# ethz-asl/multipoint

Measured on AMD Instinct MI355X. Metric: image-pairs/sec (detect+desc+match) @ 480x640, higher is better.
Workload: dtype f32

## Files before the change

### multipoint_amd/csrc/api.hip

```cpp
#include "host.h"

using namespace mp_host;

namespace {

bool debug_switch(const char* key, int* value = nullptr, int dflt = 1)
{
    const char* e = getenv("MP_DEBUG");
    if (!e) return false;
    const size_t kl = std::strlen(key);
    for (const char* q = e; *q;) {
        while (*q == ',' || *q == ' ') ++q;
        const char* end = q;
        while (*end && *end != ',') ++end;
        if ((size_t)(end - q) >= kl && std::strncmp(q, key, kl) == 0 && (q[kl] == '=' || q + kl == end || q[kl] == ' ')) {
            if (value) *value = q[kl] == '=' ? atoi(q + kl + 1) : dflt;
            return true;
        }
        q = end;
    }
    return false;
}

int kfd_num_xcc(const char* bus_id)
// ... 7 lines not shown
        FILE* f = fopen(path, "r");
        if (!f) { if (node > 8) break; else continue; }
        char key[64]; unsigned long long val = 0, loc = ~0ull, domain = 0, xcc = 0, simd = 0;
        while (fscanf(f, "%63s %llu", key, &val) == 2) {
            if (!strcmp(key, "location_id")) loc = val;
            else if (!strcmp(key, "domain")) domain = val;
            else if (!strcmp(key, "num_xcc")) xcc = val;
            else if (!strcmp(key, "simd_count")) simd = val;
        }
        fclose(f);
        if (simd > 0 && loc == want && domain == dom) return (int)xcc;
    }
    return 0;
}

}

extern "C" {

const char* mp_version(void) { return "multipoint_hip 0.1 (gfx950)"; }

const char* mp_last_error(const mp_handle* h) { return h ? h->err.c_str() : g_create_error.c_str(); }

int mp_device_shape(const mp_handle* h, int* compute_units, int* xcds, int* persistent_workgroups)
{
    if (!h) return MP_EINVAL;
    if (compute_units) *compute_units = h->ncu;
    if (xcds) *xcds = 1 << h->xcd_shift;
    if (persistent_workgroups) *persistent_workgroups = (int)persistent_grid(1ll << 40, h->ncu, h->xcd_shift);
    return MP_OK;
}

int mp_create(mp_handle** out, int device)
{
    mp_handle* h = nullptr;
    if (!out) return fail(h, MP_EINVAL, "mp_create: out is NULL");
    *out = nullptr;
    int ndev = 0;
    MP_HIP(hipGetDeviceCount(&ndev));
    if (device < 0 || device >= ndev)
        return fail(h, MP_EINVAL, "mp_create: device " + std::to_string(device) + " not available (" +
                                      std::to_string(ndev) + " HIP devices visible)");
    MP_HIP(hipSetDevice(device));
    {
        static const char* const legacy[] = {"MP_NO_WINOGRAD", "MP_WINO43", "MP_WINO43_GEN", "MP_NO_FUSE", "MP_NO_FUSE43", "MP_NO_HEAD_FUSE",
            "MP_NO_PLANAR", "MP_PLANAR", "MP_NO_PERSIST", "MP_PERSIST_MIN_ITEMS", "MP_SPLITK_MAX", "MP_F16_NO_RES", "MP_F16_NO_FUSE1",
            "MP_F16_RES_GROUPS", "MP_NCU", "MP_NXCD", "MP_POST_OVERLAP", "MP_NO_VIN", "MP_NO_POOL_FIRST"};
        static bool warned = false;
        for (const char* k : legacy)
            if (!warned && getenv(k)) {
                warned = true;
                fprintf(stderr, "libmultipoint_hip: the environment variable %s is no longer read (nor are the other MP_* kernel switches): "
                                "use MP_DEBUG=key[=value],... -- the keys are listed in csrc/api.hip (debug_switch)\n", k);
            }
    }
    hipDeviceProp_t prop;
    MP_HIP(hipGetDeviceProperties(&prop, device));
    if (std::strncmp(prop.gcnArchName, "gfx950", 6) != 0)
        return fail(h, MP_EINVAL, std::string("mp_create: kernels are built for gfx950 only, device is ") +
                                      prop.gcnArchName);
    int ncu = prop.multiProcessorCount, nxcd = 0;
    {
        char bus[64] = {0};
        if (hipDeviceGetPCIBusId(bus, sizeof bus, device) == hipSuccess) nxcd = kfd_num_xcc(bus);
        if (nxcd <= 0) nxcd = ncu >= 32 ? ncu / 32 : 1;
        int v = 0;
        if (debug_switch("ncu", &v) && v > 0 && v <= ncu) ncu = v;
        if (debug_switch("nxcd", &v) && v > 0) nxcd = v;
    }
    if (ncu < 1 || nxcd < 1 || (nxcd & (nxcd - 1)) != 0 || nxcd > ncu)
        return fail(h, MP_EINVAL, "mp_create: unsupported machine shape: " + std::to_string(ncu) + " compute units in " +
                                      std::to_string(nxcd) + " XCDs (the XCD count must be a power of two <= the CU count)");
    int xcd_shift = 0;
    while ((1 << xcd_shift) < nxcd) ++xcd_shift;
    DebugSwitches d;
    int v = 0;
    d.winograd = !debug_switch("no_winograd");
    if (debug_switch("wino43", &v) && v == 0) d.wino43 = false;
    if (debug_switch("wino43_gen", &v) && v >= 0 && v <= 2) d.wino43_gen = v;
    d.fuse_first = !debug_switch("no_fuse");
    d.fuse43 = !debug_switch("no_fuse43");
    d.head_fuse = !debug_switch("no_head_fuse");
    d.vin = !debug_switch("no_vin");
    d.planar = !debug_switch("no_planar");
    d.xplanar = d.planar && !debug_switch("no_xplanar");
    if (debug_switch("persist_min_items", &v) && v > 0) d.persist = v;
    if (debug_switch("no_persist")) d.persist = 0;
    if (debug_switch("splitk_max", &v) && v >= 1 && v <= 8) d.splitk_max = v;
    d.f16_res = !debug_switch("f16_no_res");
    d.f16_fuse1 = !debug_switch("f16_no_fuse1");
    if (debug_switch("f16_res_groups", &v) && v == 2) d.f16_res_groups = 2;
    mp_handle* hh = new mp_handle(device, ncu, xcd_shift, d);
    if (hipHostMalloc(reinterpret_cast<void**>(&hh->pinned), 4096) != hipSuccess) {
        delete hh;
        return fail(h, MP_ENOMEM, "mp_create: hipHostMalloc failed");
    }
    *out = hh;
    return MP_OK;
}

void mp_destroy(mp_handle* h)
{
    if (!h) return;
    (void)hipSetDevice(h->device);
    int* pinned = h->pinned;
    const std::vector<ProfEntry> events = std::move(h->prof_entries);
    delete h;
    if (pinned) (void)hipHostFree(pinned);
    for (auto& e : events) { (void)hipEventDestroy(e.a); (void)hipEventDestroy(e.b); }
}

int mp_profile_enable(mp_handle* h, int enable)
{
    if (!h) return MP_EINVAL;
    h->prof = enable != 0;
    h->prof_used = 0;
    return MP_OK;
}

int mp_profile_read(mp_handle* h, const char** names, float* ms, double* flop, int capacity, int* n)
{
    if (!h || !n) return MP_EINVAL;
    *n = 0;
    for (size_t i = 0; i < h->prof_used && (int)i < capacity; ++i) {
        ProfEntry& e = h->prof_entries[i];
        MP_HIP(hipEventSynchronize(e.b));
        float t = 0.f;
        MP_HIP(hipEventElapsedTime(&t, e.a, e.b));
        if (names) names[i] = e.name;
        if (ms) ms[i] = t;
        if (flop) flop[i] = e.flop;
        ++*n;
    }
    h->prof_used = 0;
    return MP_OK;
}

}
```

### multipoint_amd/csrc/conv_wino43.hip

```cpp
#include "mp_common.h"
#include "mp_device.h"
#include "mp_tile.h"

#include <algorithm>
#include <type_traits>

MP_TIMING_TABLE(g_timing_q, 256 * 8, mp_debug_read_timing_wino43)
MP_TIMING_HEIGHT(g_timing_q_sel, 480, mp_debug_select_height_wino43)

namespace {

constexpr int NPIX = 18 * 34;
constexpr int UC4 = 4;
constexpr int VB4 = UC4 * 32 * 36;
constexpr int UB4 = UC4 * 64 * 36;
constexpr int NRB = (NPIX + 63) / 64;
constexpr int RB4 = NRB * 64 * 4;
constexpr int SW4 = 8 * 36 * 2;


template <int LEAD = 0>
__device__ __forceinline__ void dma16(const float* sbase, unsigned voff_bytes, unsigned lds_byte)
{
    lds_dma<4, LEAD, 0>(sbase, voff_bytes, lds_byte);
}

template <bool POOL, bool BNF, int TC4, bool F1, bool SPLIT = false, bool VIN = false>
__global__ __launch_bounds__(512, 2) void conv_wino43_kernel(const ConvParams p)
{
    static_assert(!(F1 && SPLIT), "the fused first block is never split");
    static_assert(!(VIN && (F1 || SPLIT)), "pre-transformed input: plain launches only");
    constexpr int TR4 = 32 / TC4;
    constexpr int OY = 4 * TR4, OX = 4 * TC4;
    constexpr int PY = OY + 2, PX = OX + 2;
    static_assert(PY * PX == NPIX, "item shape");
    __shared__ __attribute__((aligned(16))) float Vs[(VIN ? 4 : 2) * VB4];
    __shared__ __attribute__((aligned(16))) float Us[2 * UB4];
    __shared__ __attribute__((aligned(16))) float raw[VIN ? 256 : 3 * RB4 + 256];
    __shared__ __attribute__((aligned(16))) float scr[VIN ? 4 : 8 * SW4];
    __shared__ __attribute__((aligned(16))) float prm[(POOL && !SPLIT ? 6 : 3) * 64];

    const int tid = threadIdx.x;
    const int lane = tid & 63;
    const int wave = __builtin_amdgcn_readfirstlane(tid >> 6);
    const int tb = wave & 1, cb = wave >> 1;
    const int NC = SPLIT ? (p.cin / UC4) >> p.ks_shift : p.cin / UC4;

    const XcdRange xr = xcd_range(p.nitems, p.xcd_shift);
    const int stride = xr.stride, item_end = xr.item_end;
    int item = xr.item;
    if (item >= item_end) return;

    struct Where { int slice, img, y0, x0, tile; const float* in_base; };
    auto decode = [&](int it) __attribute__((always_inline)) -> Where {
        Where w{};
        const int tile = (int)udiv((unsigned)it, p.magic_slices, (unsigned)p.nslices);
        w.slice = it - tile * p.nslices;
        w.tile = tile;
        const int trow = (int)udiv((unsigned)tile, p.magic_tx, (unsigned)p.tiles_x);
        const int tx = tile - trow * p.tiles_x;
        const int bi = (int)udiv((unsigned)trow, p.magic_ty, (unsigned)p.tiles_y);
        const int ty = trow - bi * p.tiles_y;
        w.img = p.img_list ? p.img_list[bi] : bi;
        w.y0 = ty * OY; w.x0 = tx * OX;
        w.in_base = p.in_planar ? p.in + (long long)w.img * (p.cin / 4) * p.H * p.W * 4
                                : p.in + (long long)w.img * p.H * p.W * p.in_cstride + p.in_coff;
        if constexpr (SPLIT)
            w.in_base += (long long)((w.slice & ((1 << p.ks_shift) - 1)) * NC) * (p.in_planar ? (long long)p.H * p.W * 4 : UC4);
        return w;
    };

    const int pix_stride = p.in_planar ? 4 : p.in_cstride;
    const long long unit_stride = p.in_planar ? (long long)p.H * p.W * 4 : UC4;
    const int x_shift = p.in_planar == MP_LAYOUT_XPLANAR ? 2 : 0, x_mask = p.in_planar == MP_LAYOUT_XPLANAR ? 3 : 0;
    const int row_stride = p.W * pix_stride;
    auto pixel_off = [&](int y, int x) __attribute__((always_inline)) -> int {
        return y * row_stride + (x >> x_shift) * pix_stride + (x & x_mask) * p.W;
    };
    unsigned rvoff[2];
    bool roff_rel = false;
    auto raw_offsets = [&](const Where& w) __attribute__((always_inline)) -> const float* {
        const bool interior = (w.y0 >= 1) && (w.y0 + OY < p.H) && (w.x0 >= 1) && (w.x0 + OX < p.W);
        if (interior) {
            if (!roff_rel) {
#pragma unroll
                for (int j = 0; j < 2; ++j) {
                    const int f = (wave + 8 * j) * 64 + lane;
                    const int py = f / PX, px = f - py * PX;
                    rvoff[j] = (f < NPIX) ? (unsigned)pixel_off(py, px + x_mask) * 4u : 0u;
                }
                roff_rel = true;
            }
            return w.in_base + pixel_off(w.y0 - 1, w.x0 - 1 - x_mask);
        }
        roff_rel = false;
#pragma unroll
        for (int j = 0; j < 2; ++j) {
            const int f = (wave + 8 * j) * 64 + lane;
            const int py = f / PX, px = f - py * PX;
            unsigned off = 0;
            if (f < NPIX) {
                const int gy = reflect_clamp(w.y0 + py - 1, p.H), gx = reflect_clamp(w.x0 + px - 1, p.W);
                off = (unsigned)pixel_off(gy, gx) * 4u;
            }
            rvoff[j] = off;
        }
        return w.in_base;
    };
    const unsigned raw_lds = lds_addr(raw), us_lds = lds_addr(Us);
    const unsigned raw_m0 = raw_lds + (unsigned)wave * 1024u;
    const unsigned raw_dummy = raw_lds + 3u * RB4 * 4u;
    auto raw_dma = [&](const float* src, unsigned boff_bytes, int j) __attribute__((always_inline)) {
        const unsigned dst = j == 0 ? raw_m0 + boff_bytes : (wave + 8 < NRB ? raw_m0 + 8192u + boff_bytes : raw_dummy);
        dma16(src, rvoff[j], dst);
    };
    int u_first, u_cnt;
    if constexpr (F1) {
        constexpr int cnt_[8] = {3, 3, 6, 6, 4, 4, 5, 5}, first_[8] = {0, 3, 14, 20, 6, 10, 26, 31};
        u_cnt = 3; u_first = 0;
#pragma unroll
        for (int w = 0; w < 8; ++w) { u_cnt = wave == w ? cnt_[w] : u_cnt; u_first = wave == w ? first_[w] : u_first; }
    } else {
        u_cnt = wave < 4 ? 5 : 4; u_first = wave < 4 ? 5 * wave : 20 + 4 * (wave - 4);
    }
    auto u_dma_site = [&](const float* ub, int buf, int site) __attribute__((always_inline)) {
        if constexpr (VIN) {
#pragma unroll
            for (int i = 3 * site; i < (site ? 5 : 3); ++i) {
                int b = wave + 8 * i;
                b = b < 36 ? b : 35;
                dma16(ub + b * 256, (unsigned)lane * 16u, us_lds + (unsigned)(buf * UB4 + b * 256) * 4u);
            }
            return;
        }
#pragma unroll
        for (int k = 3 * site; k < 3 * site + 3; ++k)
            if (k < u_cnt) {
                const int b = u_first + k;
                dma16<1>(ub + b * 256, (unsigned)lane * 16u, us_lds + (unsigned)(buf * UB4 + b * 256) * 4u);
            }
    };
// ... 315 lines not shown
                    acc[s] = __builtin_amdgcn_mfma_f32_16x16x4f32(af[g % 3][e], bf[g % 3][e], FIRST ? zero4 : acc[s], 0, 0, 0);
                    __builtin_amdgcn_sched_barrier(0);
                    if constexpr (!VIN) { if (e != 2) tf_at(g, e, vb); }
                    if constexpr (F1) prod_at(g, e, vb);
                    if (e == 0) {
                        af[(g + 2) % 3] = *reinterpret_cast<const f32x4*>(g + 2 < 9 ? &ur[4 * (g + 2)] : &urn[4 * (g - 7)]);
                        bf[(g + 2) % 3] = *reinterpret_cast<const f32x4*>(g + 2 < 9 ? &vr[4 * (g + 2)] : &vrn[4 * (g - 7)]);
                    } else if (e == 1) {
                        if (g == 7) u_dma_site(un2, vb, 0);
                        else if (g == 8) u_dma_site(un2, vb, 1);
                        else if (g == 0) { if constexpr (VIN) v_dma(vcur, (vs + 3) & 3, 0); else if constexpr (!F1) raw_dma(rsrc, rd_byte, 0); }
                        else if (g == 1) { if constexpr (VIN) v_dma(vcur, (vs + 3) & 3, 1); else if constexpr (!F1) raw_dma(rsrc, rd_byte, 1); }
                        else if (g == 2) { if constexpr (VIN) v_dma(vcur, (vs + 3) & 3, 2); }
                    } else if (e == 2) {
                        if constexpr (!VIN) tf_at(g, 2, vb);
                    } else {
                        if (g == 6) {
#ifdef MP_TIMING
                            t_b0 = __builtin_amdgcn_s_memtime();
#endif
                            if constexpr (F1) asm volatile("s_waitcnt vmcnt(0) lgkmcnt(0)" ::: "memory");
                            else if constexpr (VIN) asm volatile("s_waitcnt vmcnt(3) lgkmcnt(0)" ::: "memory");
                            else asm volatile("s_waitcnt vmcnt(2) lgkmcnt(0)" ::: "memory");
#ifdef MP_TIMING
                            t_b1 = __builtin_amdgcn_s_memtime();
#endif
                            __syncthreads();
#ifdef MP_TIMING
                            tsum[4] += __builtin_amdgcn_s_memtime() - t_b1;
#endif
                        }
                    }
                    __builtin_amdgcn_sched_barrier(0);
                }
            }
            MP_CLOCK(t_u1);
            MP_CLOCK_ADD(0, t_u0, t_u1);
            MP_CLOCK_ADD(1, t_b0, t_b1);
        };
        auto unit = [&](const int c, auto first_tag, auto vb_tag, auto vs_tag) __attribute__((always_inline)) {
            unit_body(c, first_tag, vb_tag, vs_tag);
            if constexpr (VIN) {
                v_advance();
            } else if constexpr (F1) {
                prod_advance();
            } else {
                ld_advance();
                const unsigned ro = 3u * RB4 * 4u - rd_byte - rt_byte;
                rd_byte = rt_byte; rt_byte = ro;
            }
        };
        using VB0 = std::integral_constant<int, 0>;
        using VB1 = std::integral_constant<int, 1>;
        using VS2 = std::integral_constant<int, 2>;
        using VS3 = std::integral_constant<int, 3>;
        if constexpr (VIN) {
            unit(0, std::true_type{}, VB0{}, VB0{});
            for (int c = 1; c + 3 < NC; c += 4) {
                unit(c, std::false_type{}, VB1{}, VB1{});
                unit(c + 1, std::false_type{}, VB0{}, VS2{});
                unit(c + 2, std::false_type{}, VB1{}, VS3{});
                unit(c + 3, std::false_type{}, VB0{}, VB0{});
            }
            unit(NC - 3, std::false_type{}, VB1{}, VB1{});
            unit(NC - 2, std::false_type{}, VB0{}, VS2{});
            unit(NC - 1, std::false_type{}, VB1{}, VS3{});
        } else {
        unit(0, std::true_type{}, VB0{}, VB0{});
        for (int c = 1; c + 1 < NC; c += 2) {
            unit(c, std::false_type{}, VB1{}, VB1{});
            unit(c + 1, std::false_type{}, VB0{}, VB0{});
        }
        unit(NC - 1, std::false_type{}, VB1{}, VB1{});
        }

        MP_CLOCK(t_e0);
        MP_CLOCK_ADD(3, t_item, t_e0);
        if constexpr (F1) { if (item_next + stride < item_end) patch_dma(decode(item_next + stride), cur_par); }
        const int tl = tb * 16 + (lane & 15);
        const int cl = cb * 16 + 4 * (lane >> 4);
        const f32x4 b4 = *reinterpret_cast<const f32x4*>(&prm[cl]);
        const f32x4 s4 = *reinterpret_cast<const f32x4*>(&prm[64 + cl]);
        const f32x4 t4 = *reinterpret_cast<const f32x4*>(&prm[128 + cl]);
        const int oy = cur.y0 + 4 * (tl / TC4), ox = cur.x0 + 4 * (tl % TC4);
        const int ch0 = (SPLIT ? cur.slice >> p.ks_shift : cur.slice) * 64 + cl;
        const int cs = p.out_cstride;
        constexpr int NO = POOL ? 2 : 4;
        f32x2 keep[NO][NO];
        if constexpr (SPLIT) {
            unsigned long long* const part = reinterpret_cast<unsigned long long*>(p.split_scratch) + (long long)item * (2 * 16 * 512) + tid;
#pragma unroll
            for (int h = 0; h < 2; ++h) {
                f32x2 tcol[4][6];
#pragma unroll
                for (int j = 0; j < 6; ++j) {
                    f32x2 m[6], y[4];
#pragma unroll
                    for (int i = 0; i < 6; ++i) m[i] = f32x2{acc[6 * i + j][2 * h], acc[6 * i + j][2 * h + 1]};
                    at6s(m, y);
#pragma unroll
                    for (int a = 0; a < 4; ++a) tcol[a][j] = y[a];
                }
#pragma unroll
                for (int a = 0; a < 4; ++a) {
                    f32x2 y[4];
                    at6s(tcol[a], y);
#pragma unroll
                    for (int b = 0; b < 4; ++b)
                        part[(h * 16 + a * 4 + b) * 512] = __builtin_bit_cast(unsigned long long, y[b]);
                }
            }
        }
        if constexpr (!SPLIT) {
#pragma unroll
        for (int h = 0; h < 2; ++h) {
            f32x2 tcol[4][6];
            if constexpr (!SPLIT) {
#pragma unroll
            for (int j = 0; j < 6; ++j) {
                f32x2 m[6], y[4];
#pragma unroll
                for (int i = 0; i < 6; ++i) m[i] = f32x2{acc[6 * i + j][2 * h], acc[6 * i + j][2 * h + 1]};
                at6s(m, y);
#pragma unroll
                for (int a = 0; a < 4; ++a) tcol[a][j] = y[a];
            }
            }
            const f32x2 bb = {b4[2 * h], b4[2 * h + 1]}, ss = {s4[2 * h], s4[2 * h + 1]}, tt = {t4[2 * h], t4[2 * h + 1]};
            f32x2 res[NO][NO];
            if constexpr (POOL) {
                const f32x4 g4 = *reinterpret_cast<const f32x4*>(&prm[192 + cl]);
                const f32x4 lo4 = *reinterpret_cast<const f32x4*>(&prm[256 + cl]), hi4 = *reinterpret_cast<const f32x4*>(&prm[320 + cl]);
                const f32x2 gg = {g4[2 * h], g4[2 * h + 1]};
                const f32x2 gb = bb * gg;
                constexpr float A1 = (float)MP_W43_A, A2 = A1 * A1, A3 = A2 * A1, A4 = A2 * A2;
                const f32x2 gk[5] = {gg, gg * f32x2{A1, A1}, gg * f32x2{A2, A2}, gg * f32x2{A3, A3}, gg * f32x2{A4, A4}};
                f32x2 xv[4][4];
#pragma unroll
                for (int a = 0; a < 4; ++a) {
                    f32x2 y[4];
                    at6s(tcol[a], y);
#pragma unroll
                    for (int b = 0; b < 4; ++b) {
                        const int e = (a == 1 ? 1 : a == 2 ? 2 : 0) + (b == 1 ? 1 : b == 2 ? 2 : 0);
                        xv[a][b] = __builtin_elementwise_fma(y[b], gk[e], gb);
                    }
                }
#pragma unroll
                for (int a = 0; a < NO; ++a)
#pragma unroll
                    for (int b = 0; b < NO; ++b) {
                        f32x2 m;
#pragma unroll
                        for (int r = 0; r < 2; ++r)
                            m[r] = fmaxf(fmaxf(xv[2 * a][2 * b][r], xv[2 * a][2 * b + 1][r]), fmaxf(xv[2 * a + 1][2 * b][r], xv[2 * a + 1][2 * b + 1][r]));
                        if (BNF) {
                            m = __builtin_elementwise_fma(m, ss, tt);
                            m = f32x2{relu_bits(m[0]), relu_bits(m[1])};
                        } else {
#pragma unroll
                            for (int r = 0; r < 2; ++r)
                                asm("v_med3_i32 %0, %1, %2, %3" : "=v"(m[r]) : "v"(m[r]), "v"(lo4[2 * h + r]), "v"(hi4[2 * h + r]));
                            m = __builtin_elementwise_fma(m, ss, tt);
                        }
                        res[a][b] = m;
                    }
            } else {
            f32x2 yv[4][4];
#pragma unroll
            for (int a = 0; a < 4; ++a) {
                f32x2 y[4];
                at6s(tcol[a], y);
#pragma unroll
                for (int b = 0; b < 4; ++b) {
                    f32x2 v = w43_add_bias(y[b], a, b, bb);
                    if (BNF) { v = v * ss + tt; v = f32x2{relu_bits(v[0]), relu_bits(v[1])}; }
                    else { v = f32x2{relu_bits(v[0]), relu_bits(v[1])}; v = v * ss + tt; }
                    yv[a][b] = v;
                }
            }
#pragma unroll
            for (int a = 0; a < NO; ++a)
#pragma unroll
                for (int b = 0; b < NO; ++b) res[a][b] = yv[a][b];
            }
            if (h == 0) {
#pragma unroll
                for (int a = 0; a < NO; ++a)
#pragma unroll
                    for (int b = 0; b < NO; ++b) keep[a][b] = res[a][b];
            } else {
                const int Ho = POOL ? p.H >> 1 : p.H, Wo = POOL ? p.W >> 1 : p.W;
                const int py0 = POOL ? oy >> 1 : oy, px0 = POOL ? ox >> 1 : ox;
                const bool xpl = !POOL && p.out_planar == MP_LAYOUT_XPLANAR;
                char* const img_base = reinterpret_cast<char*>(
                    p.out_planar ? p.out + (long long)cur.img * (p.cout / 4) * Ho * Wo * 4
                                 : p.out + (long long)cur.img * Ho * Wo * cs + p.out_coff);
                const unsigned ps = xpl ? (unsigned)Wo * 4u : p.out_planar ? 16u : (unsigned)cs * 4u;
                const unsigned rs = p.out_planar ? (unsigned)Wo * 16u : (unsigned)Wo * ps;
                const unsigned o0 = xpl ? (unsigned)(((ch0 >> 2) * Ho + py0) * Wo * 4 + px0) * 4u
                                  : p.out_planar ? (unsigned)(((ch0 >> 2) * Ho + py0) * Wo + px0) * 16u
                                                 : (unsigned)((py0 * Wo + px0) * cs + ch0) * 4u;
                if (oy < p.H && ox < p.W && ch0 < p.cout) {
#pragma unroll
                    for (int a = 0; a < NO; ++a)
#pragma unroll
                        for (int b = 0; b < NO; ++b) {
                            const f32x4 v = {keep[a][b][0], keep[a][b][1], res[a][b][0], res[a][b][1]};
                            *reinterpret_cast<f32x4*>(img_base + (o0 + (unsigned)a * rs + (unsigned)b * ps)) = v;
                        }
                }
            }
        }
        }
        MP_CLOCK(t_e1);
        MP_CLOCK_ADD(2, t_e0, t_e1);
#ifdef MP_TIMING
        tsum[7] += 1;
        if (!has_next && tid == 0 && t_on)
            for (int i = 0; i < 8; ++i) g_timing_q[blockIdx.x * 8 + i] = tsum[i];
#endif
        if (!has_next) { dma_wait(); return; }
        if (next_slice != cur.slice) {
            __syncthreads();
            load_prm(next_slice);
        }
        item = item_next;
        cur = decode(item);
        cur_par ^= 1;
        up = unext;
    }
}

template <int TC4>
__global__ __launch_bounds__(256) void wino43_vprod_kernel(const ConvParams p, long long ntb)
{
    constexpr int TR4 = 32 / TC4, OY = 4 * TR4, OX = 4 * TC4;
    __shared__ __attribute__((aligned(16))) float st[19456];
    const int ncp = p.cin >> 1, NC = p.cin / UC4;
    const int TL = 256 / ncp;
    const int RS = TL * 36 + 4;
    const int groups = 32 / TL;
    const int tid = threadIdx.x;
    const int cp = tid % ncp, tlc = tid / ncp;
    const long long tb = (long long)blockIdx.x / groups;
    const int t0 = ((int)((long long)blockIdx.x % groups)) * TL, t = t0 + tlc;
    (void)ntb;
    const int tx = (int)(tb % p.tiles_x);
    const long long trow = tb / p.tiles_x;
    const int ty = (int)(trow % p.tiles_y);
    const int bi = (int)(trow / p.tiles_y);
    const int img = p.img_list ? p.img_list[bi] : bi;
    const int wy = ty * OY + 4 * (t / TC4) - 1, wx = tx * OX + 4 * (t % TC4) - 1;
    const float* const base = p.in + (long long)img * p.H * p.W * p.in_cstride + p.in_coff + 2 * cp;
    int gx[6];
#pragma unroll
    for (int j = 0; j < 6; ++j) gx[j] = reflect_clamp(wx + j, p.W);
    f32x2 r[6][6];
#pragma unroll
    for (int j = 0; j < 6; ++j) {
        f32x2 d[6], o[6];
#pragma unroll
        for (int i = 0; i < 6; ++i)
            d[i] = *reinterpret_cast<const f32x2*>(base + ((long long)reflect_clamp(wy + i, p.H) * p.W + gx[j]) * p.in_cstride);
        bt6(d, o);
#pragma unroll
        for (int i = 0; i < 6; ++i) r[i][j] = o[i];
    }
    float* const dst0 = st + (2 * cp) * RS + tlc * 36;
    float* const dst1 = dst0 + RS;
#pragma unroll
    for (int i = 0; i < 6; i += 2) {
        f32x2 a[6], b[6];
        bt6(r[i], a);
        bt6(r[i + 1], b);
        *reinterpret_cast<f32x4*>(dst0 + 6 * i) = f32x4{a[0][0], a[1][0], a[2][0], a[3][0]};
        *reinterpret_cast<f32x4*>(dst0 + 6 * i + 4) = f32x4{a[4][0], a[5][0], b[0][0], b[1][0]};
        *reinterpret_cast<f32x4*>(dst0 + 6 * i + 8) = f32x4{b[2][0], b[3][0], b[4][0], b[5][0]};
        *reinterpret_cast<f32x4*>(dst1 + 6 * i) = f32x4{a[0][1], a[1][1], a[2][1], a[3][1]};
        *reinterpret_cast<f32x4*>(dst1 + 6 * i + 4) = f32x4{a[4][1], a[5][1], b[0][1], b[1][1]};
        *reinterpret_cast<f32x4*>(dst1 + 6 * i + 8) = f32x4{b[2][1], b[3][1], b[4][1], b[5][1]};
    }
    __syncthreads();
    const int q4 = TL * 9, total4 = p.cin * q4;
    float* const gbase = p.vglobal + (tb * NC * 4 * 32 + t0) * 36;
    for (int i = tid; i < total4; i += 256) {
        const int row = i / q4, w = i - row * q4;
        *reinterpret_cast<f32x4*>(gbase + (long long)row * (32 * 36) + w * 4) = *reinterpret_cast<const f32x4*>(st + row * RS + w * 4);
    }
}

template <bool POOL, int TC4, bool F1 = false, bool SPLIT = false>
int launch_q(const ConvParams& p, hipStream_t s)
{
    constexpr int OY = 4 * (32 / TC4), OX = 4 * TC4;
    ConvParams q = p;
    if (SPLIT) q.nslices = p.nslices << p.ks_shift;
    q.tiles_x = (p.W + OX - 1) / OX; q.tiles_y = (p.H + OY - 1) / OY;
    const long long nitems = (long long)p.B * q.tiles_x * q.tiles_y * q.nslices;
    if (nitems <= 0) return 0;
    if (tile_items(q, nitems)) return 1;
    const unsigned grid = persistent_grid(nitems, p.ncu, p.xcd_shift);
    const ConvParams& pp = q;
    if (p.bn_first) hipLaunchKernelGGL((conv_wino43_kernel<POOL, true, TC4, F1, SPLIT>), dim3(grid), dim3(512), 0, s, pp);
    else hipLaunchKernelGGL((conv_wino43_kernel<POOL, false, TC4, F1, SPLIT>), dim3(grid), dim3(512), 0, s, pp);
    return 0;
}

template <int TC4>
int launch_vin(const ConvParams& p, hipStream_t s)
{
    constexpr int OY = 4 * (32 / TC4), OX = 4 * TC4;
    ConvParams q = p;
    q.tiles_x = (p.W + OX - 1) / OX; q.tiles_y = (p.H + OY - 1) / OY;
    const long long ntb = (long long)p.B * q.tiles_x * q.tiles_y, nitems = ntb * q.nslices;
    if (nitems <= 0) return 0;
    if (tile_items(q, nitems)) return 1;
    const ConvParams& pp = q;
    const int tl = 256 / (p.cin / 2);
    hipLaunchKernelGGL((wino43_vprod_kernel<TC4>), dim3((unsigned)(ntb * (32 / tl))), dim3(256), 0, s, pp, ntb);
    const unsigned grid = persistent_grid(nitems, p.ncu, p.xcd_shift);
    if (p.bn_first) hipLaunchKernelGGL((conv_wino43_kernel<false, true, TC4, false, false, true>), dim3(grid), dim3(512), 0, s, pp);
    else hipLaunchKernelGGL((conv_wino43_kernel<false, false, TC4, false, false, true>), dim3(grid), dim3(512), 0, s, pp);
    return 0;
}

template <bool POOL, bool SPLIT = false>
int launch_shape(const ConvParams& p, hipStream_t s)
{
    const long long wide = (long long)((p.W + 31) / 32) * ((p.H + 15) / 16), tall = (long long)((p.W + 15) / 16) * ((p.H + 31) / 32);
    return tall < wide ? launch_q<POOL, 4, false, SPLIT>(p, s) : launch_q<POOL, 8, false, SPLIT>(p, s);
}

}

bool conv_wino43_supports(const ConvParams& p)
{
    return !p.pad_zero && p.cin % 8 == 0 && p.cout % 4 == 0 && p.H % 4 == 0 && p.W % 4 == 0 && p.H >= 4 && p.W >= 4 &&
           p.in_cstride % 4 == 0 && p.in_coff % 4 == 0 && p.out_cstride % 4 == 0 && p.out_coff % 4 == 0;
}

long long conv_wino43_vglobal_floats(const ConvParams& p)
{
    const long long wide = (long long)((p.W + 31) / 32) * ((p.H + 15) / 16), tall = (long long)((p.W + 15) / 16) * ((p.H + 31) / 32);
    return (long long)p.B * std::min(wide, tall) * (p.cin / UC4) * VB4;
}

long long conv_wino43_items(const ConvParams& p)
{
    const long long wide = (long long)((p.W + 31) / 32) * ((p.H + 15) / 16), tall = (long long)((p.W + 15) / 16) * ((p.H + 31) / 32);
    return (long long)p.B * std::min(wide, tall) * p.nslices;
}

int launch_conv_wino43(const ConvParams& p, bool pool, hipStream_t s, bool fuse_first)
{
    if (p.out_planar == MP_LAYOUT_XPLANAR && pool) return 2;
    if ((p.in_planar == MP_LAYOUT_XPLANAR || p.out_planar == MP_LAYOUT_XPLANAR) && p.ks_shift > 0) return 2;
    if (fuse_first) return pool && p.cin == 64 ? launch_q<true, 8, true>(p, s) : 2;
    if (p.vglobal) {
        if (pool || p.ks_shift > 0 || p.cin % 16 != 0 || p.in_planar || p.cin > 256 || 256 % (p.cin / 2) != 0 || (p.cin / 2) < 8) return 2;
        const long long wide = (long long)((p.W + 31) / 32) * ((p.H + 15) / 16), tall = (long long)((p.W + 15) / 16) * ((p.H + 31) / 32);
        return tall < wide ? launch_vin<4>(p, s) : launch_vin<8>(p, s);
    }
    if (p.ks_shift > 0) {
        const int ncs = (p.cin / 4) >> p.ks_shift;
        if (ncs < 4 || (ncs & 1) || (ncs << p.ks_shift) * 4 != p.cin || !p.split_scratch) return 2;
        const int rc = pool ? launch_shape<true, true>(p, s) : launch_shape<false, true>(p, s);
        return rc ? rc : launch_split_reduce(p, 1, pool, s);
    }
    return pool ? launch_shape<true>(p, s) : launch_shape<false>(p, s);
}
```

### multipoint_amd/csrc/forward.hip

```cpp
#include "host.h"

using namespace mp_host;

namespace {

int pick_mbw(int H, int W)
{
    long long best = -1;
    int arg = 32;
    for (int mbw : {32, 16, 8}) {
        const int tw = mbw, th = 256 / mbw;
        const long long area = (long long)((H + th - 1) / th) * th * ((W + tw - 1) / tw) * tw;
        if (best < 0 || area < best) { best = area; arg = mbw; }
    }
    return arg;
}

void prof_begin(mp_handle* h, const char* name, double flop, hipStream_t s)
{
    if (!h->prof) return;
    if (h->prof_used == h->prof_entries.size()) {
        ProfEntry e{};
        (void)hipEventCreate(&e.a); (void)hipEventCreate(&e.b);
        h->prof_entries.push_back(e);
// ... 76 lines not shown
    EncoderPlan P;
    if (h->cfg.mixed_precision) {
        const ConvLayer& L0 = E.conv[0];
        P.conv[0].fuse_first = h->dbg.f16_res && h->dbg.f16_fuse1 && h->cfg.reflection_pad && !E.first_pool && L0.pool &&
                               L0.cin == 64 && L0.cout == 64 && L0.nslices == 1;
        for (int i = 0; i < E.nconv; ++i) P.conv[i].kernel = f16_kind(h, E.conv[i], E.conv[i].cin, 0, P.conv[i].fuse_first);
        return P;
    }
    for (int i = 0, hh = E.first_pool ? H / 2 : H, ww = E.first_pool ? W / 2 : W; i < E.nconv; ++i) {
        const ConvLayer& L = E.conv[i];
        ConvLaunch& c = P.conv[i];
        c.kernel = wino43_kind(h, L, hh, ww, L.cin, 0, L.cout, 0);
        if (i == 0) {
            const bool fuse43 = c.kernel == Kernel::wino43 && h->dbg.fuse43 && L.pool && L.cin == 64 && L.cout == 64 &&
                                h->cfg.channel_version == 0 && L.u43pack_f1;
            c.fuse_first = h->dbg.fuse_first && h->cfg.channel_version == 0 && !E.first_pool && (h->policy.direct || fuse43);
        }
        const bool producer = i == 0 ? !E.first_pool : P.conv[i - 1].kernel != Kernel::direct && E.conv[i - 1].pool;
        c.in_planar = h->dbg.planar && c.kernel != Kernel::direct && producer ? MP_LAYOUT_PLANAR : MP_LAYOUT_NHWC;
        plan_split_vin(h, L, nb, hh, ww, fwd_batch, c);
        if (i > 0 && h->dbg.xplanar && !E.conv[i - 1].pool && P.conv[i - 1].kernel == Kernel::wino43 && P.conv[i - 1].ks_shift == 0 &&
            c.kernel == Kernel::wino43 && c.ks_shift == 0 && !c.vin)
            c.in_planar = MP_LAYOUT_XPLANAR;
        if (i > 0) P.conv[i - 1].out_planar = c.in_planar;
        if (L.pool) { hh /= 2; ww /= 2; }
    }
    return P;
}


template <typename P, typename T>
int conv_geometry(const mp_handle* h, const ConvLayer& L, P& p, const T* in, int in_cstride, int in_coff, T* out, int out_cstride,
                  int out_coff, int B, int H, int W)
{
    p.in = in; p.out = out; p.B = B; p.H = H; p.W = W;
    p.in_cstride = in_cstride; p.in_coff = in_coff; p.cin = L.cin;
    p.out_cstride = out_cstride; p.out_coff = out_coff; p.cout = L.cout; p.nslices = L.nslices;
    p.pad_zero = h->cfg.reflection_pad ? 0 : 1; p.bn_first = h->cfg.bn_first;
    p.ncu = h->ncu; p.xcd_shift = h->xcd_shift;
    const int mbw = L.taps == 9 ? pick_mbw(H, W) : 32, th = 256 / mbw;
    if (L.taps == 9) { p.tiles_x = (W + mbw - 1) / mbw; p.tiles_y = (H + th - 1) / th; }
    else p.total_px = (long long)B * H * W;
    return mbw;
}

template <typename P, typename T>
void conv1_geometry(const mp_handle* h, P& c1, const float* images, T* out, int B, int H, int W)
{
    c1.in = images; c1.out = out; c1.B = B; c1.H = H; c1.W = W;
    c1.pad_zero = h->cfg.reflection_pad ? 0 : 1; c1.bn_first = h->cfg.bn_first;
}

template <typename T>
int run_conv(mp_handle* h, const ConvLayer& L, const ConvLaunch& c, const T* in, int in_cstride, int in_coff, T* out,
             int out_cstride, int out_coff, int B, int H, int W, const int* img_list, hipStream_t s,
             const FirstLayer* first = nullptr, const float* images = nullptr)
{
    constexpr bool f16 = std::is_same<T, _Float16>::value;
    typename std::conditional<f16, ConvParamsH, ConvParams>::type p{};
    const int mbw = conv_geometry(h, L, p, in, in_cstride, in_coff, out, out_cstride, out_coff, B, H, W);
    p.scale = L.scale; p.shift = L.shift; p.img_list = img_list;
    if (c.fuse_first) {
        p.img = images; p.w1 = f16 ? first->w_h : first->w; p.b1 = f16 ? first->bias_h : first->bias;
        p.s1 = first->scale; p.t1 = first->shift;
    }
    if constexpr (f16) {
        p.wpack = L.wpack_h; p.bias = L.bias_h;
        p.dummy = static_cast<_Float16*>(h->f16_dummy.p);
        p.res_groups = h->dbg.f16_res_groups;
    } else {
        p.wpack = c.kernel == Kernel::direct ? L.wpack : L.u43pack; p.bias = L.bias;
        p.relu = L.relu ? 1 : 0;
        p.persist = h->dbg.persist;
        p.in_planar = c.in_planar; p.out_planar = c.out_planar;
        if (c.fuse_first && c.kernel != Kernel::direct) {
            p.wpack = L.u43pack_f1; p.bias = L.bias_f1; p.w1 = first->w_f1; p.b1 = first->bias_f1; p.s1 = nullptr; p.t1 = nullptr;
        }
        if (c.ks_shift) {
            const int rc = ensure(h, h->split_ws, (size_t)(conv_wino43_items(p) << c.ks_shift) * (2 * 16 * 512 * 8));
            if (rc) return rc;
            p.ks_shift = c.ks_shift; p.split_scratch = static_cast<float*>(h->split_ws.p);
        }
        if (c.vin) {
            if (ensure(h, h->vin_ws, (size_t)conv_wino43_vglobal_floats(p) * 4) == MP_OK) p.vglobal = static_cast<float*>(h->vin_ws.p);
            else { (void)hipGetLastError(); h->err.clear(); }
        }
    }
    prof_begin(h, c.fuse_first ? "enc.conv1+2" : L.name,
               2.0 * L.taps * L.cin * L.cout * (double)B * H * W + (c.fuse_first ? 2.0 * 9 * 64 * (double)B * H * W : 0.0), s);
    int big = 0;
    if constexpr (f16) {
        if (c.kernel == Kernel::f16_res) {
            big = launch_conv_f16_res(p, mbw, L.pool, s);
        } else if (c.kernel == Kernel::f16_res_slices) {
            for (int sl = 0; sl < L.nslices && !big; ++sl) {
                ConvParamsH q = p;
                q.wpack = p.wpack + (size_t)sl * 36 * 2 * 64 * 8;
                q.bias = p.bias + 64 * sl; q.scale = p.scale + 64 * sl; q.shift = p.shift + 64 * sl;
                q.out_coff = out_coff + 64 * sl; q.cout = 64; q.nslices = 1;
                big = conv_f16_res_supports(q, L.taps) ? launch_conv_f16_res(q, mbw, L.pool, s) : 2;
            }
        } else {
            big = launch_conv_f16(p, L.taps, mbw, L.pool, s);
        }
    } else {
        big = c.kernel == Kernel::wino43b ? launch_conv_wino43b(p, L.pool, s)
            : c.kernel == Kernel::wino43  ? launch_conv_wino43(p, L.pool, s, c.fuse_first)
                                          : launch_conv_mfma(p, L.taps, mbw, L.pool, c.fuse_first, s);
    }
    prof_end(h, s);
    return big ? launch_failed(h, big, L.name, B, H, W) : MP_OK;
}

template <typename T>
void run_first(mp_handle* h, const Encoder& E, bool out_planar, const float* images, T* out, int B, int H, int W,
               const int* img_list, hipStream_t s)
{
    constexpr bool f16 = std::is_same<T, _Float16>::value;
    typename std::conditional<f16, Conv1ParamsH, Conv1Params>::type c1{};
    conv1_geometry(h, c1, images, out, B, H, W);
    c1.w = f16 ? E.first.w_h : E.first.w; c1.bias = f16 ? E.first.bias_h : E.first.bias;
    c1.scale = E.first.scale; c1.shift = E.first.shift; c1.img_list = img_list;
    c1.pool = E.first_pool ? 1 : 0;
    prof_begin(h, "enc.conv1", 2.0 * 9 * 64 * (double)B * H * W, s);
    if constexpr (f16) {
        launch_conv_first_f16(c1, s);
    } else {
        c1.channels = E.first.channels; c1.out_planar = out_planar ? 1 : 0;
        launch_conv_first(c1, s);
    }
    prof_end(h, s);
}

struct FwdWorkspace { size_t P, Q, Lg, X, R, lists, bytes; };
FwdWorkspace fwd_workspace(bool f16, int B, int H, int W)
{
    const size_t el = f16 ? 2 : 4, px = (size_t)B * H * W, npx = px / 64;
    FwdWorkspace w{};
    w.Q = w.P + px * 64 * el;
    w.Lg = w.Q + px * 16 * el;
    w.X = w.Lg + npx * (f16 ? 128 : 80) * el;
    w.R = w.X + npx * 128 * el;
    w.lists = w.R + (f16 ? npx * 256 * el : 0);
    w.bytes = w.lists + 2 * 1024 * 4 + 256;
    return w;
}

struct ImageRoute {
    int counts[2] = {0, 0};
    std::vector<int> ids;
};

ImageRoute route_images(const mp_handle* h, const unsigned char* is_optical, int B)
{
    ImageRoute r;
    if (!h->cfg.multispectral) { r.counts[0] = B; return r; }
    r.ids.assign(1024, 0);
    for (int b = 0; b < B; ++b) {
        if (is_optical[b]) r.ids[512 + r.counts[1]++] = b;
        else r.ids[r.counts[0]++] = b;
    }
    return r;
}

template <typename T>
int run_forward(mp_handle* h, const float* images, const ImageRoute& route, int B, int H, int W, float* prob, float* logits, float* desc,
// ... 329 lines not shown
```

### multipoint_amd/csrc/host.h

```cpp
#pragma once
#include "../../include/multipoint_hip.h"
#include "mp_common.h"

#include <cmath>
#include <cstdio>
#include <cstdlib>
#include <cstring>
#include <string>
#include <type_traits>
#include <vector>

namespace mp_host {

inline std::string g_create_error;

struct DevBuf {
    void* p = nullptr;
    size_t bytes = 0;
    DevBuf(void* p_ = nullptr, size_t bytes_ = 0) : p(p_), bytes(bytes_) {}
    DevBuf(DevBuf&& o) noexcept : p(o.p), bytes(o.bytes) { o.p = nullptr; o.bytes = 0; }
    ~DevBuf() { if (p) (void)hipFree(p); }
};

struct ConvLayer {
    const char* name = "";
    float *wpack = nullptr, *bias = nullptr, *scale = nullptr, *shift = nullptr;
    float* u43pack = nullptr;
    float *u43pack_f1 = nullptr, *bias_f1 = nullptr;
    _Float16* wpack_h = nullptr;
    float* bias_h = nullptr;
    int cin = 0, cout = 0, taps = 9, nslices = 0;
    bool pool = false, relu = true;
};

struct FirstLayer {
    int channels = 64;
    float *w = nullptr, *bias = nullptr, *scale = nullptr, *shift = nullptr;
    float *w_h = nullptr, *bias_h = nullptr;
    float *w_f1 = nullptr, *bias_f1 = nullptr;
};

struct Encoder {
    FirstLayer first;
    ConvLayer conv[7];
    int nconv = 7;
    bool first_pool = false;
};

struct BnLayer {
    std::string name;
    int channels = 0;
    float *gamma = nullptr, *beta = nullptr;
    long long offset = 0;
};

struct ProfEntry {
    const char* name;
    hipEvent_t a, b;
    double flop;
};

struct DebugSwitches {
    bool winograd = true, wino43 = true, fuse_first = true, fuse43 = true, head_fuse = true, vin = true, planar = true;
    bool xplanar = true, f16_res = true, f16_fuse1 = true;
    int wino43_gen = 0, persist = 8, splitk_max = 8, f16_res_groups = 3;
};

struct ConvPolicy {
    bool direct = false;
    bool wino43 = true;
    int wino43_gen = 0;
    int splitk_max = 8;
};

}

struct mp_handle {
    mp_handle(int device_, int ncu_, int xcd_shift_, const mp_host::DebugSwitches& dbg_)
        : device(device_), ncu(ncu_), xcd_shift(xcd_shift_), dbg(dbg_) {}
    const int device;
    const int ncu, xcd_shift;
    const mp_host::DebugSwitches dbg;
    std::string err;
    bool loaded = false;
    mp_model_config cfg{};
    mp_host::ConvPolicy policy;
    std::vector<mp_host::DevBuf> weights;
    mp_host::Encoder enc[2];
    mp_host::ConvLayer heads3, det1, desc1;
    mp_host::DevBuf fwd_ws;
    mp_host::DevBuf nms_ws;
    mp_host::DevBuf match_ws;
    mp_host::DevBuf metrics_ws;
    mp_host::DevBuf split_ws;
    mp_host::DevBuf vin_ws;
    mp_host::DevBuf bs_ws;
    std::vector<mp_host::BnLayer> bn_layers;
    float* bn_ident = nullptr;
    mp_host::DevBuf nms_state;
    mp_host::DevBuf kp_scratch;
    mp_host::DevBuf nms_total;
    int last_nms_rounds = 0;
    mp_host::DevBuf tie_state;
    float tie_eps = 6e-5f;
    int tie_min = 4;
    int tie_last_B = 0;
    mp_host::DevBuf tie_pairs;
    int tie_pairs_min = 16;
    int head_channels = 256;
    mp_host::DevBuf f16_dummy;
    int* pinned = nullptr;
    bool prof = false;
    bool head_fallback_noted = false;
    std::vector<mp_host::ProfEntry> prof_entries;
    size_t prof_used = 0;
};

namespace mp_host {

inline int fail(mp_handle* h, int code, const std::string& msg)
{
    if (h) h->err = msg; else g_create_error = msg;
    return code;
}

#define MP_HIP(expr)                                                                          \
    do {                                                                                      \
        hipError_t _e = (expr);                                                               \
        if (_e != hipSuccess)                                                                 \
            return fail(h, MP_EHIP, std::string(#expr) + ": " + hipGetErrorString(_e));       \
    } while (0)

inline int ensure(mp_handle* h, DevBuf& b, size_t bytes)
{
    if (b.bytes >= bytes) return MP_OK;
    if (b.p) { MP_HIP(hipFree(b.p)); b.p = nullptr; b.bytes = 0; }
    hipError_t e = hipMalloc(&b.p, bytes);
    if (e != hipSuccess) {
        b.p = nullptr;
        return fail(h, MP_ENOMEM, "hipMalloc(" + std::to_string(bytes) + " B): " + hipGetErrorString(e));
    }
    b.bytes = bytes;
    return MP_OK;
}

inline int ensure_zeroed(mp_handle* h, DevBuf& b, size_t bytes, hipStream_t s)
{
// ... 14 lines not shown
```

### multipoint_amd/csrc/mp_common.h

```cpp
#pragma once
#include <hip/hip_runtime.h>
#include <stdint.h>

typedef float f32x16 __attribute__((ext_vector_type(16)));
typedef float f32x4 __attribute__((ext_vector_type(4)));
typedef float f32x2 __attribute__((ext_vector_type(2)));

#define MP_WAVE 64

enum { MP_LAYOUT_NHWC = 0, MP_LAYOUT_PLANAR = 1, MP_LAYOUT_XPLANAR = 2 };

struct ConvParams {
    const float* in;
    float* out;
    const float* wpack;
    const float* bias;
    const float* scale;
    const float* shift;
    const int* img_list;
    const float* img;
    const float *w1, *b1, *s1, *t1;
    int B, H, W;
    int in_cstride, in_coff, cin;
    int out_cstride, out_coff, cout;
    int nslices;
    int tiles_x, tiles_y;
    int pad_zero;
    int bn_first;
    int relu;
    long long total_px;
    unsigned magic_slices, magic_tx, magic_ty;
    int nitems;
    int persist;
    int in_planar, out_planar;
    int ncu, xcd_shift;
    int ks_shift;
    float* split_scratch;
    float* vglobal;
};

struct XcdRange { int item, item_end, stride; };
__device__ __forceinline__ XcdRange xcd_range(int nitems, int xcd_shift)
{
    const int nxcd = 1 << xcd_shift;
    const int per_xcd = (nitems + nxcd - 1) >> xcd_shift;
    const int xcd = (int)blockIdx.x & (nxcd - 1);
    XcdRange r;
    r.stride = (int)gridDim.x >> xcd_shift;
    r.item_end = min((xcd + 1) * per_xcd, nitems);
    r.item = xcd * per_xcd + ((int)blockIdx.x >> xcd_shift);
    return r;
}
inline unsigned persistent_grid(long long nitems, int ncu, int xcd_shift, int per_cu = 1)
{
    const long long nxcd = 1ll << xcd_shift;
    const long long full = ((long long)ncu * per_cu) / nxcd * nxcd;
    const long long need = (nitems + nxcd - 1) / nxcd * nxcd;
    return (unsigned)(need < full ? need : full);
}

struct Conv1Params {
    const float* in;
    float* out;
    const float* w;
    const float* bias; const float* scale; const float* shift;
    const int* img_list;
    int B, H, W;
    int pad_zero, bn_first;
    int channels;
    int out_planar;
    int pool;
};

int launch_conv_mfma(const ConvParams& p, int taps, int mbw, bool pool, bool fuse1, hipStream_t s);
void launch_conv_first(const Conv1Params& p, hipStream_t s);
int launch_conv_mfma_linear(const ConvParams& p, int mbw, hipStream_t s);
void launch_conv_first_linear(const Conv1Params& p, hipStream_t s);
#ifndef MP_W43_A
#define MP_W43_A 0.75
#endif
#ifndef MP_W43_B
#define MP_W43_B 1.5
#endif
constexpr unsigned long long pk_const2(double lo, double hi)
{
    return (unsigned long long)__builtin_bit_cast(unsigned, (float)lo) | ((unsigned long long)__builtin_bit_cast(unsigned, (float)hi) << 32);
}
constexpr double W43A = MP_W43_A, W43B = MP_W43_B;
constexpr unsigned long long K_AB = pk_const2(W43A, W43B), K_BA = pk_const2(W43B, W43A), K_A2B2 = pk_const2(W43A * W43A, W43B * W43B),
                             K_B2A2 = pk_const2(W43B * W43B, W43A * W43A),
                             K_PS = pk_const2(W43A * W43A * W43B * W43B, W43A * W43A + W43B * W43B);
static_assert((double)(float)(W43A * W43A * W43B * W43B) == W43A * W43A * W43B * W43B && (double)(float)(W43A * W43A + W43B * W43B) ==
              W43A * W43A + W43B * W43B, "the transform coefficients must be exact in fp32");
template <int HI>
__device__ __forceinline__ f32x2 pk_fma_k(f32x2 a, unsigned long long k, f32x2 c)
{
    f32x2 d;
    if (HI) asm("v_pk_fma_f32 %0, %1, %2, %3 op_sel:[0,1,0] op_sel_hi:[1,1,1]" : "=v"(d) : "v"(a), "s"(k), "v"(c));
    else asm("v_pk_fma_f32 %0, %1, %2, %3 op_sel:[0,0,0] op_sel_hi:[1,0,1]" : "=v"(d) : "v"(a), "s"(k), "v"(c));
    return d;
}
template <int HI>
__device__ __forceinline__ f32x2 pk_fnma_k(f32x2 a, unsigned long long k, f32x2 c)
{
    f32x2 d;
    if (HI) asm("v_pk_fma_f32 %0, %1, %2, %3 op_sel:[0,1,0] op_sel_hi:[1,1,1] neg_lo:[1,0,0] neg_hi:[1,0,0]" : "=v"(d) : "v"(a), "s"(k), "v"(c));
    else asm("v_pk_fma_f32 %0, %1, %2, %3 op_sel:[0,0,0] op_sel_hi:[1,0,1] neg_lo:[1,0,0] neg_hi:[1,0,0]" : "=v"(d) : "v"(a), "s"(k), "v"(c));
    return d;
}
__device__ __forceinline__ void bt6(const f32x2 d[6], f32x2 r[6])
{
    const f32x2 t0 = pk_fnma_k<1>(d[2], K_A2B2, d[4]);
// ... 213 lines not shown
```

### multipoint_amd/csrc/mp_tile.h

```cpp
#pragma once
#include "mp_common.h"

#include <algorithm>

template <typename P>
inline int tile_items(P& q, long long nitems)
{
    auto magic = [](int d) -> unsigned { return d <= 1 ? 0u : (unsigned)((0x100000000ull / (unsigned)d) + 1ull); };
    q.magic_slices = magic(q.nslices); q.magic_tx = magic(q.tiles_x); q.magic_ty = magic(q.tiles_y);
    const long long dmax = std::max(std::max(q.nslices, q.tiles_x), q.tiles_y);
    if (nitems * dmax >= 0x100000000ll) return 1;
    q.nitems = (int)nitems;
    return 0;
}

__device__ __forceinline__ unsigned udiv(unsigned n, unsigned magic, unsigned d) { return d == 1 ? n : __umulhi(n, magic); }

template <typename T>
struct TileWhere { int slice, img, y0, x0; long long px0; const T* in_base; };

template <typename T, int TAPS, int TH, int TW, bool SLICED = true, typename P>
__device__ __forceinline__ TileWhere<T> tile_decode(const P& p, int it)
{
    TileWhere<T> w{};
    int tile = it;
    if constexpr (SLICED) {
        tile = (int)udiv((unsigned)it, p.magic_slices, (unsigned)p.nslices);
        w.slice = it - tile * p.nslices;
    }
    if constexpr (TAPS == 9) {
        const int trow = (int)udiv((unsigned)tile, p.magic_tx, (unsigned)p.tiles_x);
        const int tx = tile - trow * p.tiles_x;
        const int bi = (int)udiv((unsigned)trow, p.magic_ty, (unsigned)p.tiles_y);
        const int ty = trow - bi * p.tiles_y;
        w.img = p.img_list ? p.img_list[bi] : bi;
        w.y0 = ty * TH; w.x0 = tx * TW;
        w.in_base = p.in + (long long)w.img * p.H * p.W * p.in_cstride + p.in_coff;
    } else {
        w.px0 = (long long)tile * 256;
        w.in_base = p.in + w.px0 * p.in_cstride + p.in_coff;
    }
    return w;
}
```

Baseline: 3427.

## Pack Winograd 4x3 VIN tiles densely across images to remove edge padding waste

In the Winograd F(4,3) path with global transformed input (VIN), the conv now enumerates 4x4 output tiles as one flat index across all images instead of rectangular 32-tile blocks per image. Each block holds 32 consecutive tiles, so partially filled edge blocks are largely removed and the transform workspace and item count shrink. Each lane computes its own image and tile coordinates, with a per-lane image offset on store and masking for tail lanes. This adds per-lane index math and less regular store addresses in exchange for fewer wasted tiles. It is on by default and can be disabled with a debug switch.

Result: no change. 3443, median of 6 (+0.5%).

```diff
diff --git a/multipoint_amd/csrc/api.hip b/multipoint_amd/csrc/api.hip
--- a/multipoint_amd/csrc/api.hip
+++ b/multipoint_amd/csrc/api.hip
@@ -113,6 +113,7 @@
     d.fuse43 = !debug_switch("no_fuse43");
     d.head_fuse = !debug_switch("no_head_fuse");
     d.vin = !debug_switch("no_vin");
+    d.dense_vin = !debug_switch("no_dense_vin");
     d.planar = !debug_switch("no_planar");
     d.xplanar = d.planar && !debug_switch("no_xplanar");
     if (debug_switch("persist_min_items", &v) && v > 0) d.persist = v;
diff --git a/multipoint_amd/csrc/conv_wino43.hip b/multipoint_amd/csrc/conv_wino43.hip
--- a/multipoint_amd/csrc/conv_wino43.hip
+++ b/multipoint_amd/csrc/conv_wino43.hip
@@ -57,6 +57,7 @@
         const int tile = (int)udiv((unsigned)it, p.magic_slices, (unsigned)p.nslices);
         w.slice = it - tile * p.nslices;
         w.tile = tile;
+        if constexpr (VIN) { if (p.dense_total) return w; }
         const int trow = (int)udiv((unsigned)tile, p.magic_tx, (unsigned)p.tiles_x);
         const int tx = tile - trow * p.tiles_x;
         const int bi = (int)udiv((unsigned)trow, p.magic_ty, (unsigned)p.tiles_y);
@@ -538,7 +539,7 @@
         const f32x4 b4 = *reinterpret_cast<const f32x4*>(&prm[cl]);
         const f32x4 s4 = *reinterpret_cast<const f32x4*>(&prm[64 + cl]);
         const f32x4 t4 = *reinterpret_cast<const f32x4*>(&prm[128 + cl]);
-        const int oy = cur.y0 + 4 * (tl / TC4), ox = cur.x0 + 4 * (tl % TC4);
+        const int oy_item = cur.y0 + 4 * (tl / TC4), ox_item = cur.x0 + 4 * (tl % TC4);
         const int ch0 = (SPLIT ? cur.slice >> p.ks_shift : cur.slice) * 64 + cl;
         const int cs = p.out_cstride;
         constexpr int NO = POOL ? 2 : 4;
@@ -647,6 +648,17 @@
                     for (int b = 0; b < NO; ++b) keep[a][b] = res[a][b];
             } else {
                 const int Ho = POOL ? p.H >> 1 : p.H, Wo = POOL ? p.W >> 1 : p.W;
+                int oy = oy_item, ox = ox_item;
+                unsigned lane_img = 0u;
+                bool real = true;
+                if constexpr (VIN) {
+                    if (p.dense_total) {
+                        const unsigned g = (unsigned)cur.tile * 32u + (unsigned)tl, last = (unsigned)p.dense_total - 1u;
+                        const DenseTile t = dense_tile(p, min(g, last));
+                        oy = 4 * t.ty; ox = 4 * t.tx; real = g <= last;
+                        lane_img = (unsigned)t.img * ((unsigned)(p.out_planar ? (p.cout / 4) * Ho * Wo * 4 : Ho * Wo * cs) * 4u);
+                    }
+                }
                 const int py0 = POOL ? oy >> 1 : oy, px0 = POOL ? ox >> 1 : ox;
                 const bool xpl = !POOL && p.out_planar == MP_LAYOUT_XPLANAR;
                 char* const img_base = reinterpret_cast<char*>(
@@ -654,10 +666,11 @@
                                  : p.out + (long long)cur.img * Ho * Wo * cs + p.out_coff);
                 const unsigned ps = xpl ? (unsigned)Wo * 4u : p.out_planar ? 16u : (unsigned)cs * 4u;
                 const unsigned rs = p.out_planar ? (unsigned)Wo * 16u : (unsigned)Wo * ps;
-                const unsigned o0 = xpl ? (unsigned)(((ch0 >> 2) * Ho + py0) * Wo * 4 + px0) * 4u
-                                  : p.out_planar ? (unsigned)(((ch0 >> 2) * Ho + py0) * Wo + px0) * 16u
-                                                 : (unsigned)((py0 * Wo + px0) * cs + ch0) * 4u;
-                if (oy < p.H && ox < p.W && ch0 < p.cout) {
+                unsigned o0 = xpl ? (unsigned)(((ch0 >> 2) * Ho + py0) * Wo * 4 + px0) * 4u
+                            : p.out_planar ? (unsigned)(((ch0 >> 2) * Ho + py0) * Wo + px0) * 16u
+                                           : (unsigned)((py0 * Wo + px0) * cs + ch0) * 4u;
+                if constexpr (VIN) o0 += lane_img;
+                if (oy < p.H && ox < p.W && ch0 < p.cout && (!VIN || real)) {
 #pragma unroll
                     for (int a = 0; a < NO; ++a)
 #pragma unroll
@@ -702,12 +715,18 @@
     const long long tb = (long long)blockIdx.x / groups;
     const int t0 = ((int)((long long)blockIdx.x % groups)) * TL, t = t0 + tlc;
     (void)ntb;
-    const int tx = (int)(tb % p.tiles_x);
-    const long long trow = tb / p.tiles_x;
-    const int ty = (int)(trow % p.tiles_y);
-    const int bi = (int)(trow / p.tiles_y);
-    const int img = p.img_list ? p.img_list[bi] : bi;
-    const int wy = ty * OY + 4 * (t / TC4) - 1, wx = tx * OX + 4 * (t % TC4) - 1;
+    int img, wy, wx;
+    if (p.dense_total) {
+        const DenseTile d = dense_tile(p, (unsigned)min(tb * 32 + t, (long long)p.dense_total - 1));
+        img = d.img; wy = 4 * d.ty - 1; wx = 4 * d.tx - 1;
+    } else {
+        const int tx = (int)(tb % p.tiles_x);
+        const long long trow = tb / p.tiles_x;
+        const int ty = (int)(trow % p.tiles_y);
+        const int bi = (int)(trow / p.tiles_y);
+        img = p.img_list ? p.img_list[bi] : bi;
+        wy = ty * OY + 4 * (t / TC4) - 1; wx = tx * OX + 4 * (t % TC4) - 1;
+    }
     const float* const base = p.in + (long long)img * p.H * p.W * p.in_cstride + p.in_coff + 2 * cp;
     int gx[6];
 #pragma unroll
@@ -763,13 +782,31 @@
     return 0;
 }
 
+long long vin_dense_blocks(const ConvParams& p, ConvParams* q = nullptr)
+{
+    if (!p.dense_total || p.img_list || p.B <= 0) return 0;
+    const long long img_floats = p.out_planar ? (long long)(p.cout / 4) * p.H * p.W * 4 : (long long)p.H * p.W * p.out_cstride;
+    if ((long long)p.B * img_floats * 4 >= 0x100000000ll) return 0;
+    ConvParams t = p;
+    if (dense_tile_setup(t)) return 0;
+    const long long ntb = ((long long)t.dense_total + 31) / 32;
+    if (ntb * p.nslices * std::max(std::max(p.nslices, t.tiles_x), t.tiles_y) >= 0x100000000ll) return 0;
+    if (q) *q = t;
+    return ntb;
+}
+
 template <int TC4>
 int launch_vin(const ConvParams& p, hipStream_t s)
 {
     constexpr int OY = 4 * (32 / TC4), OX = 4 * TC4;
     ConvParams q = p;
-    q.tiles_x = (p.W + OX - 1) / OX; q.tiles_y = (p.H + OY - 1) / OY;
-    const long long ntb = (long long)p.B * q.tiles_x * q.tiles_y, nitems = ntb * q.nslices;
+    long long ntb = vin_dense_blocks(p, &q);
+    if (!ntb) {
+        q.dense_total = 0;
+        q.tiles_x = (p.W + OX - 1) / OX; q.tiles_y = (p.H + OY - 1) / OY;
+        ntb = (long long)p.B * q.tiles_x * q.tiles_y;
+    }
+    const long long nitems = ntb * q.nslices;
     if (nitems <= 0) return 0;
     if (tile_items(q, nitems)) return 1;
     const ConvParams& pp = q;
@@ -798,12 +835,15 @@
 
 long long conv_wino43_vglobal_floats(const ConvParams& p)
 {
+    if (const long long ntb = vin_dense_blocks(p)) return ntb * (p.cin / UC4) * VB4;
     const long long wide = (long long)((p.W + 31) / 32) * ((p.H + 15) / 16), tall = (long long)((p.W + 15) / 16) * ((p.H + 31) / 32);
     return (long long)p.B * std::min(wide, tall) * (p.cin / UC4) * VB4;
 }
 
 long long conv_wino43_items(const ConvParams& p)
 {
+    if (p.vglobal)
+        if (const long long ntb = vin_dense_blocks(p)) return ntb * p.nslices;
     const long long wide = (long long)((p.W + 31) / 32) * ((p.H + 15) / 16), tall = (long long)((p.W + 15) / 16) * ((p.H + 31) / 32);
     return (long long)p.B * std::min(wide, tall) * p.nslices;
 }
@@ -816,6 +856,7 @@
     if (p.vglobal) {
         if (pool || p.ks_shift > 0 || p.cin % 16 != 0 || p.in_planar || p.cin > 256 || 256 % (p.cin / 2) != 0 || (p.cin / 2) < 8) return 2;
         const long long wide = (long long)((p.W + 31) / 32) * ((p.H + 15) / 16), tall = (long long)((p.W + 15) / 16) * ((p.H + 31) / 32);
+        if (vin_dense_blocks(p)) return launch_vin<8>(p, s);
         return tall < wide ? launch_vin<4>(p, s) : launch_vin<8>(p, s);
     }
     if (p.ks_shift > 0) {
diff --git a/multipoint_amd/csrc/forward.hip b/multipoint_amd/csrc/forward.hip
--- a/multipoint_amd/csrc/forward.hip
+++ b/multipoint_amd/csrc/forward.hip
@@ -182,6 +182,7 @@
             p.ks_shift = c.ks_shift; p.split_scratch = static_cast<float*>(h->split_ws.p);
         }
         if (c.vin) {
+            p.dense_total = h->dbg.dense_vin ? 1 : 0;
             if (ensure(h, h->vin_ws, (size_t)conv_wino43_vglobal_floats(p) * 4) == MP_OK) p.vglobal = static_cast<float*>(h->vin_ws.p);
             else { (void)hipGetLastError(); h->err.clear(); }
         }
diff --git a/multipoint_amd/csrc/host.h b/multipoint_amd/csrc/host.h
--- a/multipoint_amd/csrc/host.h
+++ b/multipoint_amd/csrc/host.h
@@ -62,7 +62,7 @@
 
 struct DebugSwitches {
     bool winograd = true, wino43 = true, fuse_first = true, fuse43 = true, head_fuse = true, vin = true, planar = true;
-    bool xplanar = true, f16_res = true, f16_fuse1 = true;
+    bool xplanar = true, dense_vin = true, f16_res = true, f16_fuse1 = true;
     int wino43_gen = 0, persist = 8, splitk_max = 8, f16_res_groups = 3;
 };
 
diff --git a/multipoint_amd/csrc/mp_common.h b/multipoint_amd/csrc/mp_common.h
--- a/multipoint_amd/csrc/mp_common.h
+++ b/multipoint_amd/csrc/mp_common.h
@@ -28,6 +28,7 @@
     int pad_zero;
     int bn_first;
     int relu;
+    int dense_total;
     long long total_px;
     unsigned magic_slices, magic_tx, magic_ty;
     int nitems;
diff --git a/multipoint_amd/csrc/mp_tile.h b/multipoint_amd/csrc/mp_tile.h
--- a/multipoint_amd/csrc/mp_tile.h
+++ b/multipoint_amd/csrc/mp_tile.h
@@ -15,6 +15,28 @@
 }
 
 __device__ __forceinline__ unsigned udiv(unsigned n, unsigned magic, unsigned d) { return d == 1 ? n : __umulhi(n, magic); }
+
+template <typename P>
+inline int dense_tile_setup(P& q)
+{
+    const long long tx = q.W / 4, ty = q.H / 4, total = (long long)q.B * tx * ty;
+    if (total <= 0 || (total + 32) * std::max(tx, ty) >= 0x100000000ll) return 1;
+    q.tiles_x = (int)tx; q.tiles_y = (int)ty; q.dense_total = (int)total;
+    return 0;
+}
+
+struct DenseTile { int img, ty, tx; };
+template <typename P>
+__device__ __forceinline__ DenseTile dense_tile(const P& p, unsigned g)
+{
+    DenseTile t;
+    const unsigned trow = udiv(g, p.magic_tx, (unsigned)p.tiles_x);
+    t.tx = (int)(g - trow * (unsigned)p.tiles_x);
+    const unsigned bi = udiv(trow, p.magic_ty, (unsigned)p.tiles_y);
+    t.ty = (int)(trow - bi * (unsigned)p.tiles_y);
+    t.img = p.img_list ? p.img_list[bi] : (int)bi;
+    return t;
+}
 
 template <typename T>
 struct TileWhere { int slice, img, y0, x0; long long px0; const T* in_base; };
```
